# gfxdisp/FovVideoVDP

Measured on AMD Instinct MI355X. Metric: Mpixels/s (test+ref) at 4Kx60f; JOD delta vs reference, higher is better.
Workload: dtype f32

## Files before the change

fovvideovdp_amd/csrc/band2_kernel.hpp:

```cpp
#pragma once
constexpr int F2_PITCH = 54;
constexpr int F2_HL = 6;

struct Band2Args {
    L0Addr A;
    float* Gc;
    int w, h, wb, hb, wc, hc;
    int n_strips, n_chunks, kr;
    int n_big, kr2, n_frames;
    float mulA, mulB;
    const float4* csfA;
    const float4* csfB;
    float y_first, y_inv_step, ly_lo, ly_hi;
    float lg_gain, lg_k, p, q0, q1, beta, lbkg_min, cmax, lg_dmax;
    float* partialA;
    float* partialB;
    int* tickets;
    int n_items;
};

__device__ __forceinline__ v2f dpp_reduce5_pair(v2f acc, v2f v, float u0, float u1, float u3, float u4) {
    float x = acc.x, y = acc.y, l1x, l1y, r1x, r1y, ox, oy;
    asm volatile("s_nop 1\n\t"
                 "v_mov_b32_dpp %2, %8" DPP_SHR "\n\t"
                 "v_mov_b32_dpp %3, %9" DPP_SHR "\n\t"
                 "v_mov_b32_dpp %4, %8" DPP_SHL "\n\t"
                 "v_mov_b32_dpp %5, %9" DPP_SHL "\n\t"
                 "v_fmac_f32_dpp %0, %8, %12" DPP_SHL "\n\t"
                 "v_fmac_f32_dpp %1, %9, %12" DPP_SHL "\n\t"
                 "v_fmac_f32_dpp %0, %2, %10" DPP_SHR "\n\t"
                 "v_fmac_f32_dpp %1, %3, %10" DPP_SHR "\n\t"
                 "v_fmac_f32_dpp %0, %8, %11" DPP_SHR "\n\t"
                 "v_fmac_f32_dpp %1, %9, %11" DPP_SHR "\n\t"
                 "v_fmac_f32_dpp %0, %4, %13" DPP_SHL "\n\t"
                 "v_fmac_f32_dpp %1, %5, %13" DPP_SHL "\n\t"
                 "s_nop 1\n\t"
                 "v_mov_b32_dpp %6, %0 quad_perm:[0,0,2,2] row_mask:0xf bank_mask:0xf bound_ctrl:1\n\t"
                 "v_mov_b32_dpp %7, %1 quad_perm:[0,0,2,2] row_mask:0xf bank_mask:0xf bound_ctrl:1"
                 : "+v"(x), "+v"(y), "=&v"(l1x), "=&v"(l1y), "=&v"(r1x), "=&v"(r1y), "=&v"(ox), "=&v"(oy)
                 : "v"(v.x), "v"(v.y), "v"(u0), "v"(u1), "v"(u3), "v"(u4));
    return v2f{ox, oy};
}
__device__ __forceinline__ v2f dpp_expand2_taps(v2f t, v2f e, float fl, float fr) {
    float x = t.x, y = t.y, l1x, l1y, r1x, r1y;
    asm volatile("s_nop 1\n\t"
                 "v_mov_b32_dpp %2, %6" DPP_SHR "\n\t"
                 "v_mov_b32_dpp %3, %7" DPP_SHR "\n\t"
                 "v_mov_b32_dpp %4, %6" DPP_SHL "\n\t"
                 "v_mov_b32_dpp %5, %7" DPP_SHL "\n\t"
                 "v_fmac_f32_dpp %0, %2, %8" DPP_SHR "\n\t"
                 "v_fmac_f32_dpp %1, %3, %8" DPP_SHR "\n\t"
                 "v_fmac_f32_dpp %0, %4, %9" DPP_SHL "\n\t"
                 "v_fmac_f32_dpp %1, %5, %9" DPP_SHL
                 : "+v"(x), "+v"(y), "=&v"(l1x), "=&v"(l1y), "=&v"(r1x), "=&v"(r1y)
                 : "v"(e.x), "v"(e.y), "v"(fl), "v"(fr));
    return v2f{x, y};
}

constexpr int BAND2_LB = 3;

template <int P, bool INRANGE>
__device__ __forceinline__ void band2_item(const Band2Args& a, const int strip, const int chunk, const int frame, const int lane,
                                           const float4 (*s_csf)[FVVDP_LUT_N], const bool in_step = false) {
    constexpr int HP = P / 2;
    const int blk = chunk * a.n_strips + strip;

    const int w = a.w, h = a.h, wb = a.wb, hb = a.hb, wc = a.wc, hc = a.hc;
    const int J = strip * F2_PITCH - F2_HL + lane;
    const int K = J >> 1;
    const bool jeven = (lane & 1) == 0;
    const bool big = chunk < a.n_big;
    const int ka = big ? chunk * a.kr : a.n_big * a.kr + (chunk - a.n_big) * a.kr2;
    const int kb = min(ka + (big ? a.kr : a.kr2), hc);
    const int ca = 2 * ka, cb = min(2 * kb, hb);
    const bool owned = lane >= F2_HL && lane < F2_HL + F2_PITCH && J < wb;
    const int X0 = 2 * J, X1 = 2 * J + 1;
    const int xc0 = min(max(X0, 0), w - 1), xc1 = min(max(X1, 0), w - 1);
    const bool col1_ok = X1 < w;

    const float K0 = 0.05f, K1 = 0.25f, K2 = 0.4f, K3 = 0.25f, K4 = 0.05f;
    float wq0 = K0, wq1 = K1, wq2 = K2, wq3 = K3, wq4 = K4;
    if (J == 0) { wq2 += K1; wq3 += K0; wq0 = 0.0f; wq1 = 0.0f; }
    if (J == wb - 1) {
        const bool hodd = (h & 1) != 0;
        if (w & 1) { wq3 = 0.0f; wq4 = 0.0f; if (hodd) { wq2 += K3; wq1 += K4; } else { wq2 += K4; } }
        else { wq4 = 0.0f; if (hodd) { wq3 += K3; wq2 += K4; } else { wq3 += K4; } }
    }
    float uq0 = K0, uq1 = K1, uq2 = K2, uq3 = K3, uq4 = K4;
    if (K == 0) { uq2 += K1; uq3 += K0; uq0 = 0.0f; uq1 = 0.0f; }
    if (K == wc - 1) {
        const bool hodd = (hb & 1) != 0;
        if (wb & 1) { uq3 = 0.0f; uq4 = 0.0f; if (hodd) { uq2 += K3; uq1 += K4; } else { uq2 += K4; } }
        else { uq4 = 0.0f; if (hodd) { uq3 += K3; uq2 += K4; } else { uq3 += K4; } }
    }
    const bool at_l = (J <= 0), at_r = (J >= wb - 1);
    const float el = at_l ? 0.0f : 0.1f, er = at_r ? 0.0f : 0.1f;
    const float ec = 0.8f + (at_l ? 0.1f : 0.0f) + (at_r ? 0.1f : 0.0f);
    const float orr = at_r ? 0.0f : 0.5f, oc = at_r ? 1.0f : 0.5f;
    const bool k_l = (K <= 0), k_r = (K >= wc - 1);
    const float fl = (jeven && !k_l) ? 0.1f : 0.0f;
    const float fr = k_r ? 0.0f : (jeven ? 0.1f : 0.5f);
    const float fc = jeven ? (0.8f + (k_l ? 0.1f : 0.0f) + (k_r ? 0.1f : 0.0f)) : (k_r ? 1.0f : 0.5f);

    const float* Ga = l0_frame(a.A, frame);
    float* Gc = a.Gc + (size_t)frame * hc * wc * P;
    const __amdgpu_buffer_rsrc_t Gc_rsrc = level_rsrc(Gc, (unsigned int)(hc * wc * P) * 4u);

    const __amdgpu_buffer_rsrc_t Ga_rsrc = level_rsrc(const_cast<float*>(Ga), (unsigned int)(h * w * P) * 4u);
    const unsigned int col0_b = (unsigned int)xc0 * (P * 4u), col1_b = (unsigned int)xc1 * (P * 4u);
    const unsigned int row_b = (unsigned int)w * (P * 4u);
    auto load_row = [&](int r, Px<P>& p0, Px<P>& p1) {
        int rr = r < 0 ? -1 - r : (r >= h ? 2 * h - 1 - r : r);
        rr = min(max(rr, 0), h - 1);
        const unsigned int so = (unsigned int)rr * row_b;
        p0 = ld_px_buf<P>(Ga_rsrc, col0_b, so);
        p1 = ld_px_buf<P>(Ga_rsrc, col1_b, so);
    };


    Px<P> S[8][2];
    auto coarse_step = [&](auto base) -> Px<P> {
        constexpr int B = decltype(base)::value;
        Px<P>(&W0)[2] = S[(B + 0) & 7]; Px<P>(&W1)[2] = S[(B + 1) & 7]; Px<P>(&W2)[2] = S[(B + 2) & 7];
        Px<P>(&W3)[2] = S[(B + 3) & 7]; Px<P>(&W4)[2] = S[(B + 4) & 7];
        Px<P> c, va, vb;
#pragma unroll
        for (int k = 0; k < HP; ++k) {
            v2f a0 = W0[0].h[k] * K0;
            a0 = pfma(W1[0].h[k], K1, a0);
            a0 = pfma(W2[0].h[k], K2, a0);
            a0 = pfma(W3[0].h[k], K3, a0);
            va.h[k] = pfma(W4[0].h[k], K4, a0);
            v2f b0 = W0[1].h[k] * K0;
            b0 = pfma(W1[1].h[k], K1, b0);
            b0 = pfma(W2[1].h[k], K2, b0);
            b0 = pfma(W3[1].h[k], K3, b0);
            vb.h[k] = pfma(W4[1].h[k], K4, b0);
        }
#pragma unroll
        for (int k = 0; k < HP; ++k) {
            v2f acc = va.h[k] * wq2;
            acc = pfma(vb.h[k], wq3, acc);
            c.h[k] = dpp_reduce_taps(acc, va.h[k], vb.h[k], wq0, wq1, wq4);
        }
        return c;
    };
    float accA[2] = {0.0f, 0.0f}, accB[2] = {0.0f, 0.0f};
    const float lg_base = a.lg_gain;
    const float lg_mask = a.lg_gain + a.lg_k;
    const float lg_bm[2] = {__log2f(a.mulA), __log2f(a.mulB)};
    const float pb = a.p * a.beta, pb_base = lg_base * pb, b_dmax = a.beta * a.lg_dmax, y_off = -a.y_first * a.y_inv_step;

    auto tail = [&](const Px<P>& g, const Px<P>& e, bool valid, const int band, float (&acc)[2]) {
        const float lb = INRANGE ? e.h[0].y : fmaxf(e.h[0].y, a.lbkg_min);
        const float dcap = a.cmax * lb;
        v2f d[HP];
#pragma unroll
        for (int k = 0; k < HP; ++k) {
            if constexpr (INRANGE) d[k] = v2f{g.h[k].x - e.h[k].x, g.h[k].y - e.h[k].y};
            else d[k] = v2f{fminf(g.h[k].x - e.h[k].x, dcap), fminf(g.h[k].y - e.h[k].y, dcap)};
        }
        const float llb = fast_log2(lb);
        const float yq = INRANGE ? llb : __builtin_amdgcn_fmed3f(llb, a.ly_lo, a.ly_hi);
        const float t = fmaf(yq, a.y_inv_step, y_off);
        float4 r;
        float f;
        if constexpr (INRANGE) {
            r = s_csf[band][floor_to_int(t)];
            f = __builtin_amdgcn_fractf(t);
        } else {
            const float fi = __builtin_amdgcn_fmed3f(floorf(t), 0.0f, (float)(FVVDP_LUT_N - 2));
            r = s_csf[band][(int)fi];
            f = t - fi;
        }
        const float slog0 = fmaf(f, r.z, r.x), slog1 = fmaf(f, r.w, r.y);
        const float vm = valid ? 1.0f : 0.0f;
        const float lcn = lg_bm[band] - llb;
        if constexpr (HP == 2) {
            const v2f sl = v2f{slog0, slog1};
            const v2f A = pfma(sl, pb, splat(fmaf(lcn, pb, pb_base)));
            const v2f lsm = sl + splat(lcn + lg_mask);
            const v2f ldiff = v2f{fast_log2(fabsf(d[0].x - d[0].y)), fast_log2(fabsf(d[1].x - d[1].y))};
            const v2f lmin = v2f{fast_log2(fminf(fabsf(d[0].x), fabsf(d[0].y))), fast_log2(fminf(fabsf(d[1].x), fabsf(d[1].y)))};
            const v2f ldb = pfma(ldiff, pb, A);
            const v2f lm = (lmin + lsm) * v2f{a.q0, a.q1};
            const v2f one_mq = v2f{fast_exp2(lm.x), fast_exp2(lm.y)} + splat(1.0f);
            const v2f tb = pfma(v2f{fast_log2(one_mq.x), fast_log2(one_mq.y)}, -a.beta, ldb);
            const v2f bl = v2f{fminf(tb.x, b_dmax), fminf(tb.y, b_dmax)};
            const v2f term = v2f{fast_exp2(bl.x), fast_exp2(bl.y)};
            const v2f av = __builtin_elementwise_fma(term, splat(vm), v2f{acc[0], acc[1]});
            acc[0] = av.x;
            acc[1] = av.y;
        } else {
            const float dT = d[0].x, dR = d[0].y;
            const float ls = slog0 + lcn;
            const float ld = a.p * (fast_log2(fabsf(dT - dR)) + (ls + lg_base));
            const float mq = fast_exp2(a.q0 * (fast_log2(fminf(fabsf(dT), fabsf(dR))) + (ls + lg_mask)));
            const float ldd = fminf(ld - fast_log2(1.0f + mq), a.lg_dmax);
            acc[0] = fmaf(fast_exp2(a.beta * ldd), vm, acc[0]);
        }
// ... 60 lines not shown
            e0.h[k] = dpp_expand2_taps(evE.h[k] * fc, evE.h[k], fl, fr);
            e1.h[k] = dpp_expand2_taps(evO.h[k] * fc, evO.h[k], fl, fr);
        }
        tail(g0, e0, owned && row0 < hb, 1, accB);
        tail(g1, e1, owned && (row0 + 1) < hb, 1, accB);
    };

    auto stage = [&](auto basea, auto baseb, int k) {
        constexpr int BA = decltype(basea)::value, BB = decltype(baseb)::value;
        Px<P> Be, Bo;
        if (in_step) __builtin_amdgcn_s_barrier();
        {
            const int c = 2 * k;
            load_row(2 * c + 5, S[(BA + 5) & 7][0], S[(BA + 5) & 7][1]);
            load_row(2 * c + 6, S[(BA + 6) & 7][0], S[(BA + 6) & 7][1]);
            Be = coarse_step(basea);
            if (c + 1 >= hb) Be = R[4];
            if (c >= ca && c < cb) band_a_rows(basea, c, R[3], R[4], Be);
        }
        {
            const int c = 2 * k + 1;
            load_row(2 * c + 5, S[(BB + 5) & 7][0], S[(BB + 5) & 7][1]);
            load_row(2 * c + 6, S[(BB + 6) & 7][0], S[(BB + 6) & 7][1]);
            Bo = coarse_step(baseb);
            if (c + 1 >= hb) Bo = (c + 1 == hb) ? Be : R[3];
            if (c >= ca && c < cb) band_a_rows(baseb, c, R[4], Be, Bo);
        }
        R[0] = R[2];
        R[1] = R[3];
        R[2] = R[4];
        R[3] = Be;
        R[4] = Bo;
        if (k == 0) {
            R[0] = R[3];
            R[1] = R[2];
        }
        Px<P> Cn;
#pragma unroll
        for (int q = 0; q < HP; ++q) {
            v2f v = R[0].h[q] * K0;
            v = pfma(R[1].h[q], K1, v);
            v = pfma(R[2].h[q], K2, v);
            v = pfma(R[3].h[q], K3, v);
            v = pfma(R[4].h[q], K4, v);
            Cn.h[q] = dpp_reduce5_pair(v * uq2, v, uq0, uq1, uq3, uq4);
        }
        st_px(Gc_rsrc, (k >= ka && k < kb && owned && jeven && K < wc) ? (unsigned int)(k * wc + K) * (P * 4u) : FVVDP_NO_STORE, Cn);
        CH[0] = CH[1];
        CH[1] = CH[2];
        CH[2] = Cn;
        if (k == 0) CH[1] = Cn;
        const int row0 = 2 * k - 2;
        if (row0 >= ca && row0 < cb) band_b_rows(R[0], R[1], row0);
    };
    {
        int k = ks;
        for (; k + 1 <= kend; k += 2) {
            stage(I0(), I2(), k);
            stage(I4(), I6(), k + 1);
        }
        if (k <= kend) stage(I0(), I2(), k);
    }
    if (last_chunk) {
        const int row0 = 2 * hc - 2;
        CH[0] = CH[1];
        CH[1] = CH[2];
        if (row0 >= ca && row0 < cb) band_b_rows(R[2], R[3], row0);
    }

    const float a0 = wave_sum(accA[0]), a1 = wave_sum(accA[1]);
    const float b0 = wave_sum(accB[0]), b1 = wave_sum(accB[1]);
    if (lane == 0) {
        const size_t o = ((size_t)frame * (a.n_strips * a.n_chunks) + blk) * 2;
        a.partialA[o] = a0;
        a.partialA[o + 1] = a1;
        a.partialB[o] = b0;
        a.partialB[o + 1] = b1;
    }
}

#define BAND2_WPB_MAX 4

template <int P, bool INRANGE = false>
__global__ __launch_bounds__(64 * BAND2_WPB_MAX, BAND2_LB) void band2_kernel(const Band2Args a) {
    __shared__ float4 s_csf[2][FVVDP_LUT_N];
    __shared__ int s_item[2];
    const int lane = threadIdx.x & 63;
    const int wpb = (int)(blockDim.x >> 6);
    const int n_groups = a.n_strips / wpb;
    const int first = n_groups * a.n_big * a.n_frames;
    int bid;
    bool tall;
    if (a.tickets) {
        if (threadIdx.x == 0) {
#if defined(__gfx942__) || defined(__gfx950__)
            const int x = (int)__builtin_amdgcn_s_getreg((4 - 1) << 11 | 20) & 7;
#else
            const int x = (int)(blockIdx.x & 7);
#endif
            const int nbp[2] = {first, a.n_items - first};
            int item = -1, ph_found = 0;
            for (int k = 0; k < 16 && item < 0; ++k) {
                const int ph = (k == 0) ? 0 : (k == 1 ? 1 : (k < 9 ? 0 : 1));
                const int y = (k < 2) ? x : ((x + (k < 9 ? k - 1 : k - 8)) & 7);
                const int q8 = nbp[ph] >> 3, r8 = nbp[ph] & 7, cnt = q8 + (y < r8 ? 1 : 0);
                int* tk = a.tickets + ph * 8 + y;
                if (__hip_atomic_load(tk, __ATOMIC_RELAXED, __HIP_MEMORY_SCOPE_AGENT) >= cnt) continue;
                const int t = atomicAdd(tk, 1);
                if (t < cnt) { item = y * q8 + min(y, r8) + t; ph_found = ph; }
            }
            s_item[0] = item;
            s_item[1] = ph_found;
        }
        __syncthreads();
        bid = s_item[0];
        tall = s_item[1] == 0;
        if (bid < 0) return;
    } else {
        int v = (int)blockIdx.x, nb = first;
        tall = v < first;
        if (!tall) { v -= first; nb = (int)gridDim.x - first; }
        const int q8 = nb >> 3, r8 = nb & 7, x = v & 7;
        bid = x * q8 + min(x, r8) + (v >> 3);
    }
    const int group = bid % n_groups;
    bid /= n_groups;
    const int per_frame = tall ? a.n_big : a.n_chunks - a.n_big;
    const int chunk = (tall ? 0 : a.n_big) + bid % per_frame;
    const int frame = bid / per_frame;
    const int strip = group * wpb + (int)(threadIdx.x >> 6);
    if (threadIdx.x < FVVDP_LUT_N) {
        s_csf[0][threadIdx.x] = a.csfA[threadIdx.x];
        s_csf[1][threadIdx.x] = a.csfB[threadIdx.x];
    }
    __syncthreads();
    band2_item<P, INRANGE>(a, strip, chunk, frame, lane, s_csf, wpb > 1);
}
```

fovvideovdp_amd/csrc/fvvdp_hip.hip:

```cpp
#include <hip/hip_runtime.h>
#include <hip/hip_fp16.h>

#include <algorithm>
#include <cmath>
#include <cfloat>
#include <cstdarg>
#include <cstdio>
#include <cstdlib>
#include <cstring>
#include <type_traits>
#include <vector>

#include "fvvdp_hip.h"
#include "fvvdp_hip_images.h"
#include "fvvdp_hip_gaze.h"
#include "fvvdp_hip_tests.h"
#include "fvvdp_hip_ref_grad.h"
#include "fvvdp_hip_params.h"
#include "fvvdp_hip_diffmap.h"

static thread_local char g_err[512] = "";

static int fail(int code, const char* fmt, ...) {
    va_list ap;
    va_start(ap, fmt);
    vsnprintf(g_err, sizeof(g_err), fmt, ap);
    va_end(ap);
    return code;
}

#define HIP_TRY(expr)                                                                              \
    do {                                                                                           \
        hipError_t e_ = (expr);                                                                    \
        if (e_ != hipSuccess) return fail(FVVDP_EHIP, "%s failed: %s", #expr, hipGetErrorString(e_)); \
    } while (0)

extern "C" const char* fvvdp_last_error(void) { return g_err; }
int fvvdp_fail_from(int code, const char* msg) { return fail(code, "%s", msg); }

#include "device_common.hpp"
#include "temporal_kernels.hpp"
#include "temporal_launch.hpp"
#include "band_kernel.hpp"
#include "band2_kernel.hpp"
#include "aux_kernels.hpp"
#include "multigaze_kernel.hpp"
#include "multitest_kernel.hpp"
#include "still_kernels.hpp"
#include "psnr_kernel.hpp"
#include "resize_kernels.hpp"

struct CtxEnv {
    bool alloc_malloc = false;
    size_t vmm_chunk = 0;
    int probe_n = -1;
    int probe_extra = -1;
    float probe_mixed = 6.75f;
    bool inrange_off = false;
    int fuse_mode = -1;
    int band2_kr = 0, band2_kr2 = -1, band2_wpb = 0;
    int k1_ticket = -1;
    int level0_split = -1;
    int band2_ticket = -1;
    bool temporal_scalar = false;
    bool debug_variant = false;
    int gaze_group = 0;
    int band_cr = 0;
    int tests_group = 0;
    bool yuv_general = false;
};
static CtxEnv read_env() {
    CtxEnv e;
    auto num = [](const char* name, int dflt) { const char* v = getenv(name); return (v && v[0]) ? atoi(v) : dflt; };
    if (const char* v = getenv("FVVDP_ALLOC")) e.alloc_malloc = strcmp(v, "malloc") == 0;
    e.vmm_chunk = (size_t)(num("FVVDP_VMM_CHUNK_MB", 0) > 0 ? num("FVVDP_VMM_CHUNK_MB", 0) : 0) << 20;
    e.probe_n = num("FVVDP_PLACEMENT_PROBE", -1);
    e.probe_extra = num("FVVDP_PLACEMENT_EXTRA", -1);
    if (const char* v = getenv("FVVDP_PLACEMENT_MIXED_TBS")) e.probe_mixed = (float)atof(v);
    if (const char* v = getenv("FVVDP_BAND_INRANGE")) e.inrange_off = v[0] == '0';
    if (const char* v = getenv("FVVDP_BAND_FUSE")) e.fuse_mode = (v[0] == '0' || v[0] == '1') ? v[0] - '0' : -1;
    e.band2_kr = num("FVVDP_BAND2_KR", 0);
    e.band2_kr2 = num("FVVDP_BAND2_KR2", -1);
    e.band2_wpb = num("FVVDP_BAND2_WPB", 0);
    if (const char* v = getenv("FVVDP_K1_TICKET")) e.k1_ticket = v[0] != '0' ? 1 : 0;
    if (const char* v = getenv("FVVDP_BAND2_TICKET")) e.band2_ticket = v[0] != '0' ? 1 : 0;
    if (const char* v = getenv("FVVDP_LEVEL0_SPLIT")) e.level0_split = v[0] != '0' ? 1 : 0;
    e.temporal_scalar = getenv("FVVDP_TEMPORAL_SCALAR") != nullptr;
    e.debug_variant = getenv("FVVDP_DEBUG_VARIANT") != nullptr;
    e.yuv_general = getenv("FVVDP_YUV_GENERAL_MATRIX") != nullptr;
    e.gaze_group = num("FVVDP_GAZE_GROUP", 0);
    e.band_cr = num("FVVDP_BAND_CR", 0);
    e.tests_group = num("FVVDP_TESTS_GROUP", 0);
    return e;
}

struct VmmBlock {
    void* ptr;
    size_t size;
    std::vector<hipMemGenericAllocationHandle_t> handles;
};
struct fvvdp_ctx {
    CtxEnv env;
    int W = 0, H = 0, n_bands = 0, P = 0, max_frames = 0;
    fvvdp_params prm{};
    double rho_band[FVVDP_MAX_BANDS + 1]{};
    int lw[FVVDP_MAX_BANDS + 1]{}, lh[FVVDP_MAX_BANDS + 1]{};
    float* level[FVVDP_MAX_BANDS + 1]{};
    float* level0_hi = nullptr;
    int sel_phase = 9;
    int sel_n = 0;
    int sel_kept = -1;
    float sel_us[8] = {0, 0, 0, 0, 0, 0, 0, 0};
    int level0_kind = 0;
    int level0_kind_hi = -1;
    long long n_sync = 0, n_alloc = 0, n_free = 0;
    bool created = false;
    bool lum_known = false;
    int lum_state = 0;
    int lum_hold = 0;
    int lum_top = 0;
    float lum_lo = 0.0f, lum_hi = 0.0f, lum_width = 0.0f;
    float* partial = nullptr;
    long long partial_off[FVVDP_MAX_BANDS]{};
    int max_blk[FVVDP_MAX_BANDS]{};
    int* d_ticket = nullptr;
    size_t partial_floats = 0;
    float4* csf = nullptr;
    float4* csf_y = nullptr;
    bool csf_set = false;
    float y_first = 0, y_inv_step = 0, y_lo = 0, y_hi = 0;
    std::vector<float> h_lut3[2];
    float h_axes[3][FVVDP_LUT_N]{};
    float* d_axes = nullptr;
    float4* sublut[FVVDP_MAX_BANDS]{};
    float4* rmap[FVVDP_MAX_BANDS]{};
    int sub_rw[FVVDP_MAX_BANDS]{}, sub_ilo[FVVDP_MAX_BANDS]{};
    fvvdp_geom sub_geom{};
    const float* map_vx[FVVDP_MAX_BANDS]{};
    const float* map_vy[FVVDP_MAX_BANDS]{};
    const float* map_rm[FVVDP_MAX_BANDS]{};
    float map_rm_max[FVVDP_MAX_BANDS]{}, map_rm_min[FVVDP_MAX_BANDS]{};
    bool maps_set = false;
    float* slope[FVVDP_MAX_BANDS]{};
    bool sub_valid = false;
    float rho_lo = 0, rho_hi = 0, ecc_lo = 0, ecc_hi = 0;
    bool lut3_set[2] = {false, false};
    float* d_fix = nullptr;
    float* d_taps = nullptr;
    int* d_idx = nullptr;
    float* lum_buf = nullptr;
    size_t lum_floats = 0;
    float* heat[FVVDP_MAX_BANDS + 1]{};
    unsigned int* colour_ws = nullptr;
    size_t scratch = 0;
    std::vector<VmmBlock> vmm;
    long long wave_capacity = 4096;
    long long wave_capacity2 = 4096;
    bool timing = false;
    std::vector<std::pair<hipEvent_t, hipEvent_t>> ev[FVVDP_MAX_BANDS + 2];
    float t_ms[FVVDP_MAX_BANDS + 2]{};
    int t_cnt[FVVDP_MAX_BANDS + 2]{};
};

static const size_t VMM_MIN_BYTES = (size_t)16 << 20;
static const size_t VMM_BIG_BYTES = (size_t)256 << 20;

static int vmm_alloc(fvvdp_ctx* c, void** out, size_t bytes);
static void vmm_free_all(fvvdp_ctx* c);

template <typename T>
static int dev_alloc(fvvdp_ctx* c, T** p, size_t count) {
    void* q = nullptr;
    const size_t bytes = count * sizeof(T);
    if (!c->env.alloc_malloc && bytes >= VMM_MIN_BYTES && vmm_alloc(c, &q, bytes) == FVVDP_OK) {
    } else {
        q = nullptr;
        (void)hipGetLastError();
        hipError_t e = hipMalloc(&q, bytes);
        if (e != hipSuccess) return fail(FVVDP_ENOMEM, "hipMalloc(%zu bytes) failed: %s", bytes, hipGetErrorString(e));
    }
    *p = reinterpret_cast<T*>(q);
    c->scratch += bytes;
    if (c->created) c->n_alloc += 1;
    return FVVDP_OK;
}

static L0Addr level_addr(const fvvdp_ctx* c, int L, int slot0) {
    L0Addr a;
    const size_t fr = (size_t)c->lw[L] * c->lh[L] * c->P;
    a.lo = c->level[L];
    a.slot0 = slot0;
    if (L == 0 && c->level0_hi) { a.hi = c->level0_hi; a.half_stride = fr; }
    else { a.hi = c->level[L] + fr; a.half_stride = 2 * fr; }
    return a;
}

struct Timed {
    fvvdp_ctx* c;
    int id;
    hipStream_t st;
    hipEvent_t e0 = nullptr, e1 = nullptr;
    Timed(fvvdp_ctx* c_, int id_, hipStream_t st_) : c(c_), id(id_), st(st_) {
        if (c->timing) {
            (void)hipEventCreate(&e0);
            (void)hipEventCreate(&e1);
            (void)hipEventRecord(e0, st);
        }
    }
    ~Timed() {
        if (c->timing) {
// ... 35 lines not shown
        if (e == hipSuccess) mapped = (i + 1) * chunk;
    }
    hipMemAccessDesc acc;
    memset(&acc, 0, sizeof(acc));
    acc.location = prop.location;
    acc.flags = hipMemAccessFlagsProtReadWrite;
    if (e == hipSuccess) e = hipMemSetAccess(b.ptr, size, &acc, 1);
    if (e != hipSuccess) {
        if (mapped) (void)hipMemUnmap(b.ptr, mapped);
        for (auto h : b.handles) (void)hipMemRelease(h);
        (void)hipMemAddressFree(b.ptr, size);
        return fail(FVVDP_ENOMEM, "mapping %zu chunks of %zu bytes failed: %s", n, chunk, hipGetErrorString(e));
    }
    c->vmm.push_back(b);
    *out = b.ptr;
    return FVVDP_OK;
}

static bool vmm_owns(const fvvdp_ctx* c, const void* p) {
    for (const VmmBlock& b : c->vmm)
        if (b.ptr == p) return true;
    return false;
}

static void dev_free(fvvdp_ctx* c, void* p) {
    if (p && !vmm_owns(c, p)) (void)hipFree(p);
}

static void vmm_free_one(fvvdp_ctx* c, void* p) {
    for (size_t i = 0; i < c->vmm.size(); ++i)
        if (c->vmm[i].ptr == p) {
            VmmBlock& b = c->vmm[i];
            (void)hipMemUnmap(b.ptr, b.size);
            for (auto h : b.handles) (void)hipMemRelease(h);
            (void)hipMemAddressFree(b.ptr, b.size);
            c->vmm.erase(c->vmm.begin() + (long)i);
            return;
        }
}

static void vmm_free_all(fvvdp_ctx* c) {
    for (VmmBlock& b : c->vmm) {
        (void)hipMemUnmap(b.ptr, b.size);
        for (auto h : b.handles) (void)hipMemRelease(h);
        (void)hipMemAddressFree(b.ptr, b.size);
    }
    c->vmm.clear();
}

static int band_strips(int wc) { return wc <= 62 ? 1 : 1 + (wc - 62 + STRIP_J - 1) / STRIP_J; }

static int band2_strips(int wb) { return (wb + F2_PITCH - 1) / F2_PITCH; }

static void chunking2(int hc, int n_strips, int n, long long capacity, int kr_override, int& n_chunks, int& kr) {
    double best = 1e300;
    kr = hc;
    for (int cand = 1; cand <= hc; ++cand) {
        const long long chunks = (hc + cand - 1) / cand;
        const long long waves = (long long)n * n_strips * chunks;
        const long long rounds = (waves + capacity - 1) / capacity;
        const double cost = (double)rounds * (2.0 * cand + 9.0) * (1.0 + 1e-4 * (double)chunks);
        if (cost < best) { best = cost; kr = cand; }
    }
    if (kr_override >= 1) kr = kr_override > hc ? hc : kr_override;
    n_chunks = (hc + kr - 1) / kr;
}

static void chunking(int hc, int n_strips, int n, long long capacity, int& n_chunks, int& cr) {
    double best = 1e300;
    cr = hc;
    for (int cand = 2; cand <= hc || cand == 2; ++cand) {
        const int c = cand > hc ? hc : cand;
        const long long chunks = (hc + c - 1) / c;
        const long long waves = (long long)n * n_strips * chunks;
        const long long rounds = (waves + capacity - 1) / capacity;
        const double cost = (double)rounds * ((double)c + 8.0) * (1.0 + 1e-4 * (double)chunks);
        if (cost < best) { best = cost; cr = c; }
        if (cand >= hc) break;
    }
    n_chunks = (hc + cr - 1) / cr;
}

static void choose_level0(fvvdp_ctx* c);

static bool band2_takes(const fvvdp_ctx* c, int b) {
    const bool big = (long long)c->lw[b] * c->lh[b] >= 500000;
    return (big || c->env.fuse_mode == 1) && b + 1 < c->n_bands && c->lw[b + 1] >= 4 && c->lh[b + 1] >= 4 &&
           c->lw[b + 2] >= 2 && c->lh[b + 2] >= 2;
}

static void band2_plan(const fvvdp_ctx* c, int b, int plan_n, int& n_strips, int& n_chunks, int& kr, int& n_big, int& kr2_out) {
    const int hc = c->lh[b + 2];
    n_strips = band2_strips(c->lw[b + 1]);
    chunking2(hc, n_strips, plan_n, c->wave_capacity2, c->env.band2_kr, n_chunks, kr);
    n_big = n_chunks;
    kr2_out = kr;
    const long long waves = (long long)plan_n * n_strips * n_chunks;
    int kr2 = (waves >= 2 * c->wave_capacity2 && n_chunks >= 3 && kr >= 16) ? (kr + 3) / 4 : 0;
    if (c->env.band2_kr2 >= 0) kr2 = c->env.band2_kr2;
    if (kr2 >= 1 && kr2 < kr && n_chunks >= 2) {
        n_big = n_chunks - 1;
        kr2_out = kr2;
        n_chunks = n_big + (hc - n_big * kr + kr2 - 1) / kr2;
    }
}

extern "C" int fvvdp_ctx_create(fvvdp_ctx** out, int width, int height, int n_bands, int planes, int max_frames,
                                const double* h_rho_band, const fvvdp_params* prm) {
    if (!out || !prm || !h_rho_band) return fail(FVVDP_EINVAL, "null argument");
    if (planes != 2 && planes != 4) return fail(FVVDP_EINVAL, "planes must be 2 (image) or 4 (video), got %d", planes);
    if (n_bands < 1 || n_bands > FVVDP_MAX_BANDS) return fail(FVVDP_EINVAL, "n_bands %d out of range", n_bands);
    if (max_frames < 1) return fail(FVVDP_EINVAL, "max_frames must be >= 1");
    if (width < 4 || height < 4) return fail(FVVDP_EINVAL, "frame %dx%d too small", width, height);
    fvvdp_ctx* c = new fvvdp_ctx();
    c->env = read_env();
    c->W = width;
    c->H = height;
    c->n_bands = n_bands;
    c->P = planes;
    c->max_frames = max_frames;
    c->prm = *prm;
    int w = width, h = height;
    for (int i = 0; i <= n_bands; ++i) {
        c->lw[i] = w;
        c->lh[i] = h;
        c->rho_band[i] = h_rho_band[i];
        if (i < n_bands && (w < 2 || h < 2)) {
            delete c;
            return fail(FVVDP_EINVAL, "pyramid level %d is %dx%d: too many bands for this frame size", i, w, h);
        }
        w = (w + 1) / 2;
        h = (h + 1) / 2;
    }
    int rc = FVVDP_OK;
    for (int i = 0; i <= n_bands && rc == FVVDP_OK; ++i) {
        rc = dev_alloc(c, &c->level[i], (size_t)max_frames * c->lw[i] * c->lh[i] * planes);
    }
    size_t off = 0;
    for (int b = 0; b < n_bands; ++b) {
        const int n_strips = band_strips(c->lw[b + 1]);
        const int max_chunks = (c->lh[b + 1] + 1) / 2;
        c->max_blk[b] = n_strips * max_chunks;
    }
    for (int b = 0; b + 1 < n_bands; ++b) {
        const int blk2 = band2_strips(c->lw[b + 1]) * c->lh[b + 2];
        if (blk2 > c->max_blk[b]) c->max_blk[b] = blk2;
        if (blk2 > c->max_blk[b + 1]) c->max_blk[b + 1] = blk2;
    }
    for (int b = 0; b < n_bands; ++b) {
        c->partial_off[b] = (long long)off;
        off += (size_t)max_frames * c->max_blk[b] * 2;
    }
    c->partial_floats = off;
    if (rc == FVVDP_OK) rc = dev_alloc(c, &c->partial, off);
    if (rc == FVVDP_OK) {
        float* q = nullptr;
        rc = dev_alloc(c, &q, 16);
        c->d_ticket = reinterpret_cast<int*>(q);
    }
    if (rc == FVVDP_OK) rc = dev_alloc(c, &c->csf, (size_t)n_bands * FVVDP_LUT_N);
    if (rc == FVVDP_OK) rc = dev_alloc(c, &c->csf_y, (size_t)FVVDP_LUT_N);
    if (rc == FVVDP_OK) rc = dev_alloc(c, &c->d_fix, (size_t)max_frames * 2);
    if (rc == FVVDP_OK) rc = dev_alloc(c, &c->d_taps, (size_t)2 * FVVDP_MAX_TAPS);
    if (rc == FVVDP_OK) rc = dev_alloc(c, &c->d_idx, (size_t)max_frames + FVVDP_MAX_TAPS);
    if (rc != FVVDP_OK) {
        fvvdp_ctx_destroy(c);
        return rc;
    }
    {
        int dev = 0, cus = 256, per_cu = 16;
        if (hipGetDevice(&dev) == hipSuccess) {
            hipDeviceProp_t prop;
            if (hipGetDeviceProperties(&prop, dev) == hipSuccess) cus = prop.multiProcessorCount;
        }
        hipError_t e = (planes == 4)
            ? hipOccupancyMaxActiveBlocksPerMultiprocessor(&per_cu, band_kernel<4, false, 0>, 64, 0)
            : hipOccupancyMaxActiveBlocksPerMultiprocessor(&per_cu, band_kernel<2, false, 0>, 64, 0);
        if (e != hipSuccess || per_cu < 1) per_cu = 16;
        c->wave_capacity = (long long)per_cu * cus;
        int per_cu2 = 16;
        e = (planes == 4) ? hipOccupancyMaxActiveBlocksPerMultiprocessor(&per_cu2, band2_kernel<4, false>, 64, 0)
                          : hipOccupancyMaxActiveBlocksPerMultiprocessor(&per_cu2, band2_kernel<2, false>, 64, 0);
        if (e != hipSuccess || per_cu2 < 1) per_cu2 = 16;
        c->wave_capacity2 = (long long)per_cu2 * cus;
    }
    choose_level0(c);
    if (!c->level[0]) {
        fvvdp_ctx_destroy(c);
        return fail(FVVDP_ENOMEM, "no device memory for pyramid level 0");
    }
    c->created = true;
    *out = c;
    return FVVDP_OK;
}

extern "C" void fvvdp_ctx_destroy(fvvdp_ctx* c) {
    if (!c) return;
    (void)hipDeviceSynchronize();
    for (int i = 0; i <= FVVDP_MAX_BANDS; ++i)
        dev_free(c, c->level[i]);
    dev_free(c, c->level0_hi);
    dev_free(c, c->partial);
    dev_free(c, c->d_ticket);
    if (c->csf) (void)hipFree(c->csf);
    if (c->csf_y) (void)hipFree(c->csf_y);
    for (int i = 0; i <= FVVDP_MAX_BANDS; ++i)
        dev_free(c, c->heat[i]);
    if (c->colour_ws) (void)hipFree(c->colour_ws);
    if (c->d_fix) (void)hipFree(c->d_fix);
    if (c->d_taps) (void)hipFree(c->d_taps);
// ... 800 lines not shown
    hipStream_t st = reinterpret_cast<hipStream_t>(stream);
    if (fov) {
        HIP_TRY(hipMemcpyAsync(c->d_fix, h_fixation, sizeof(float) * 2 * n, hipMemcpyHostToDevice, st));
        int rc = build_sublut(c, geom, st);
        if (rc != FVVDP_OK) return rc;
    }
    FinalizeArgs fa;
    memset(&fa, 0, sizeof(fa));
    bool any_maps = false;
    if (maps)
        for (int b = 0; b < c->n_bands; ++b) any_maps = any_maps || maps[b].d_D || maps[b].d_contrast || maps[b].d_lbkg || maps[b].d_S;
    const int fuse_mode = c->env.fuse_mode;
    const bool fuse_ok = !fov && !any_maps && fuse_mode != 0;
    for (int b = 0; b < c->n_bands; ++b) {
        if (fuse_ok && band2_takes(c, b)) {
            Band2Args a;
            memset(&a, 0, sizeof(a));
            a.A = level_addr(c, b, b == 0 ? slot0 : 0);
            a.Gc = c->level[b + 2];
            a.w = c->lw[b];
            a.h = c->lh[b];
            a.wb = c->lw[b + 1];
            a.hb = c->lh[b + 1];
            a.wc = c->lw[b + 2];
            a.hc = c->lh[b + 2];
            band2_plan(c, b, plan_n, a.n_strips, a.n_chunks, a.kr, a.n_big, a.kr2);
            a.n_frames = n;
            a.mulA = (b == 0) ? 1.0f : 2.0f;
            a.mulB = 2.0f;
            a.csfA = c->csf + (size_t)b * FVVDP_LUT_N;
            a.csfB = c->csf + (size_t)(b + 1) * FVVDP_LUT_N;
            a.y_first = c->y_first;
            a.y_inv_step = c->y_inv_step;
            a.ly_lo = log2f(c->y_lo);
            a.ly_hi = log2f(c->y_hi);
            a.lg_gain = log2f(c->prm.sens_gain);
            a.lg_k = log2f(c->prm.mask_k);
            a.p = c->prm.mask_p;
            a.q0 = c->prm.mask_q[0];
            a.q1 = c->prm.mask_q[1];
            a.beta = c->prm.beta;
            a.lbkg_min = c->prm.lbkg_min;
            a.cmax = c->prm.contrast_max;
            a.lg_dmax = log2f(c->prm.d_max);
            a.partialA = c->partial + c->partial_off[b];
            a.partialB = c->partial + c->partial_off[b + 1];
            const int nblk = a.n_strips * a.n_chunks;
            if (nblk > c->max_blk[b] || nblk > c->max_blk[b + 1]) return fail(FVVDP_ESTATE, "internal: partial buffer too small");
            {
                Timed tm(c, 1 + b, st);
                const bool inrange = clamps_never_bind(c, b, 2);
                int wpb = (a.w >= 2560 && a.n_strips % BAND2_WPB_MAX == 0) ? BAND2_WPB_MAX : 1;
                { const int v = c->env.band2_wpb; if (v >= 1 && v <= BAND2_WPB_MAX && a.n_strips % v == 0) wpb = v; }
                const int n_items = (a.n_strips / wpb) * a.n_chunks * n;
                const long long waves2 = (long long)n * a.n_strips * a.n_chunks;
                bool tickets = c->d_ticket && (c->env.band2_ticket == 1 ||
                                               (c->env.band2_ticket != 0 && waves2 >= 2 * c->wave_capacity2 && wpb == BAND2_WPB_MAX && a.w >= 2560));
                if (tickets && hipMemsetAsync(c->d_ticket, 0, 16 * sizeof(int), st) != hipSuccess) { (void)hipGetLastError(); tickets = false; }
                a.n_items = n_items;
                a.tickets = tickets ? c->d_ticket : nullptr;
                const int n_wg = tickets ? ((n_items + n_items / 8 + 7) / 8 * 8) : n_items;
                const dim3 grid2((unsigned int)n_wg), block2(64 * wpb);
                if (c->env.debug_variant)
                    fprintf(stderr, "fvvdp: levels %d+%d: band2_kernel<%d, %s>, luminance range %s [%g, %g], widest plane range %g, %d waves per workgroup"
                                    ", n_strips %d, kr %d, kr2 %d, n_big %d, n_chunks %d, tickets %s\n",
                                 b, b + 1, c->P, inrange ? "true" : "false", c->lum_state == 1 ? "known" : "unknown", c->lum_lo, c->lum_hi, c->lum_width, wpb,
                                 a.n_strips, a.kr, a.kr2, a.n_big, a.n_chunks, tickets ? "on" : "off");
                if (c->P == 4) {
                    if (inrange) hipLaunchKernelGGL((band2_kernel<4, true>), grid2, block2, 0, st, a);
                    else hipLaunchKernelGGL((band2_kernel<4, false>), grid2, block2, 0, st, a);
                } else {
                    if (inrange) hipLaunchKernelGGL((band2_kernel<2, true>), grid2, block2, 0, st, a);
                    else hipLaunchKernelGGL((band2_kernel<2, false>), grid2, block2, 0, st, a);
                }
            }
            for (int bb = b; bb <= b + 1; ++bb) {
                fa.nblk[bb] = nblk;
                fa.off[bb] = c->partial_off[bb];
                fa.npx[bb] = (float)c->lw[bb] * (float)c->lh[bb];
            }
            ++b;
            continue;
        }
        BandArgs a;
        fill_band_args(c, b, slot0, plan_n, fov, geom, a);
        a.partial = c->partial + c->partial_off[b];
        bool dbg = false;
        if (maps) {
            a.dD = maps[b].d_D;
            a.dC = maps[b].d_contrast;
            a.dL = maps[b].d_lbkg;
            a.dS = maps[b].d_S;
            dbg = a.dD || a.dC || a.dL || a.dS;
        }
        const int nblk = a.n_strips * a.n_chunks;
        if (nblk > c->max_blk[b]) return fail(FVVDP_ESTATE, "internal: partial buffer too small");
        a.n_items = nblk * n;
        if (c->env.debug_variant) debug_band_line(c, b, a, n, dbg, fov);
        {
            Timed tm(c, 1 + b, st);
            if (c->P == 4) launch_band<4>(a, nblk * n, dbg, fov, st, c->slope[b]);
            else launch_band<2>(a, nblk * n, dbg, fov, st, c->slope[b]);
        }
        fa.nblk[b] = nblk;
        fa.off[b] = c->partial_off[b];
        fa.npx[b] = (float)a.w * (float)a.h;
    }
    fa.partial = c->partial;
    fa.Q = d_Q;
    fa.n_bands = c->n_bands;
    fa.n = n;
    fa.q_stride = q_stride;
    fa.q_col0 = q_col0;
    fa.tc = c->P / 2;
    fa.inv_beta = 1.0f / c->prm.beta;
    {
        Timed tm(c, 1 + c->n_bands, st);
        const int total = c->n_bands * 2 * n;
        hipLaunchKernelGGL(finalize_kernel, dim3(total), dim3(64), 0, st, fa);
    }
// ... 782 lines not shown
```

Baseline: 259,600.

## Merge adjacent band2 row chunks into multi-chunk runs chosen by a makespan planner

Lets a single band2 work item process a run of consecutive row chunks. It flushes per-chunk partial sums at the chunk seams, so the overlap and startup rows are not recomputed for each chunk. A host-side planner simulates the makespan of candidate run layouts against wave capacity and picks the best one, memoised per geometry. The ticket scheduler and the plain scheduler are generalised to up to four phases. The trade is fewer, longer items and so possibly worse load balance, plus extra host planning work on first use.

```diff
diff --git a/fovvideovdp_amd/csrc/band2_kernel.hpp b/fovvideovdp_amd/csrc/band2_kernel.hpp
--- a/fovvideovdp_amd/csrc/band2_kernel.hpp
+++ b/fovvideovdp_amd/csrc/band2_kernel.hpp
@@ -17,6 +17,8 @@
     float* partialB;
     int* tickets;
     int n_items;
+    int n_phases;
+    int run_first[BAND2_MAX_PHASES], run_len[BAND2_MAX_PHASES], run_count[BAND2_MAX_PHASES], ph_items[BAND2_MAX_PHASES];
 };
 
 __device__ __forceinline__ v2f dpp_reduce5_pair(v2f acc, v2f v, float u0, float u1, float u3, float u4) {
@@ -60,18 +62,18 @@
 constexpr int BAND2_LB = 3;
 
 template <int P, bool INRANGE>
-__device__ __forceinline__ void band2_item(const Band2Args& a, const int strip, const int chunk, const int frame, const int lane,
+__device__ __forceinline__ void band2_item(const Band2Args& a, const int strip, const int chunk, const int run_len, const int frame, const int lane,
                                            const float4 (*s_csf)[FVVDP_LUT_N], const bool in_step = false) {
     constexpr int HP = P / 2;
-    const int blk = chunk * a.n_strips + strip;
 
     const int w = a.w, h = a.h, wb = a.wb, hb = a.hb, wc = a.wc, hc = a.hc;
     const int J = strip * F2_PITCH - F2_HL + lane;
     const int K = J >> 1;
     const bool jeven = (lane & 1) == 0;
-    const bool big = chunk < a.n_big;
-    const int ka = big ? chunk * a.kr : a.n_big * a.kr + (chunk - a.n_big) * a.kr2;
-    const int kb = min(ka + (big ? a.kr : a.kr2), hc);
+    auto chunk_row0 = [&](int c) { return min(c <= a.n_big ? c * a.kr : a.n_big * a.kr + (c - a.n_big) * a.kr2, hc); };
+    const int chunk_last = chunk + run_len - 1;
+    const int ka = chunk_row0(chunk);
+    const int kb = chunk_row0(chunk_last + 1);
     const int ca = 2 * ka, cb = min(2 * kb, hb);
     const bool owned = lane >= F2_HL && lane < F2_HL + F2_PITCH && J < wb;
     const int X0 = 2 * J, X1 = 2 * J + 1;
@@ -146,6 +148,17 @@
         return c;
     };
     float accA[2] = {0.0f, 0.0f}, accB[2] = {0.0f, 0.0f};
+    auto flush = [&](float (&acc)[2], float* partial, int c) {
+        const float s0 = wave_sum(acc[0]), s1 = wave_sum(acc[1]);
+        if (lane == 0) {
+            const size_t o = ((size_t)frame * (a.n_strips * a.n_chunks) + (c * a.n_strips + strip)) * 2;
+            partial[o] = s0;
+            partial[o + 1] = s1;
+        }
+        acc[0] = 0.0f;
+        acc[1] = 0.0f;
+    };
+    int cur = chunk, seam = chunk_row0(chunk + 1);
     const float lg_base = a.lg_gain;
     const float lg_mask = a.lg_gain + a.lg_k;
     const float lg_bm[2] = {__log2f(a.mulA), __log2f(a.mulB)};
@@ -312,6 +325,14 @@
         if (k == 0) CH[1] = Cn;
         const int row0 = 2 * k - 2;
         if (row0 >= ca && row0 < cb) band_b_rows(R[0], R[1], row0);
+        if (cur < chunk_last) {
+            if (k == seam) {
+                flush(accB, a.partialB, cur);
+                ++cur;
+                seam = chunk_row0(cur + 1);
+            }
+            if (k + 1 == seam && cur < chunk_last) flush(accA, a.partialA, cur);
+        }
     };
     {
         int k = ks;
@@ -328,15 +349,8 @@
         if (row0 >= ca && row0 < cb) band_b_rows(R[2], R[3], row0);
     }
 
-    const float a0 = wave_sum(accA[0]), a1 = wave_sum(accA[1]);
-    const float b0 = wave_sum(accB[0]), b1 = wave_sum(accB[1]);
-    if (lane == 0) {
-        const size_t o = ((size_t)frame * (a.n_strips * a.n_chunks) + blk) * 2;
-        a.partialA[o] = a0;
-        a.partialA[o + 1] = a1;
-        a.partialB[o] = b0;
-        a.partialB[o + 1] = b1;
-    }
+    flush(accA, a.partialA, chunk_last);
+    flush(accB, a.partialB, chunk_last);
 }
 
 #define BAND2_WPB_MAX 4
@@ -348,9 +362,7 @@
     const int lane = threadIdx.x & 63;
     const int wpb = (int)(blockDim.x >> 6);
     const int n_groups = a.n_strips / wpb;
-    const int first = n_groups * a.n_big * a.n_frames;
-    int bid;
-    bool tall;
+    int bid, ph;
     if (a.tickets) {
         if (threadIdx.x == 0) {
 #if defined(__gfx942__) || defined(__gfx950__)
@@ -358,35 +370,37 @@
 #else
             const int x = (int)(blockIdx.x & 7);
 #endif
-            const int nbp[2] = {first, a.n_items - first};
+            const int np = a.n_phases;
             int item = -1, ph_found = 0;
-            for (int k = 0; k < 16 && item < 0; ++k) {
-                const int ph = (k == 0) ? 0 : (k == 1 ? 1 : (k < 9 ? 0 : 1));
-                const int y = (k < 2) ? x : ((x + (k < 9 ? k - 1 : k - 8)) & 7);
-                const int q8 = nbp[ph] >> 3, r8 = nbp[ph] & 7, cnt = q8 + (y < r8 ? 1 : 0);
-                int* tk = a.tickets + ph * 8 + y;
+            for (int k = 0; k < 8 * np && item < 0; ++k) {
+                const int p = k < np ? k : (k - np) / 7;
+                const int y = k < np ? x : ((x + 1 + (k - np) % 7) & 7);
+                const int nb = a.ph_items[p];
+                const int q8 = nb >> 3, r8 = nb & 7, cnt = q8 + (y < r8 ? 1 : 0);
+                int* tk = a.tickets + p * 8 + y;
                 if (__hip_atomic_load(tk, __ATOMIC_RELAXED, __HIP_MEMORY_SCOPE_AGENT) >= cnt) continue;
                 const int t = atomicAdd(tk, 1);
-                if (t < cnt) { item = y * q8 + min(y, r8) + t; ph_found = ph; }
+                if (t < cnt) { item = y * q8 + min(y, r8) + t; ph_found = p; }
             }
             s_item[0] = item;
             s_item[1] = ph_found;
         }
         __syncthreads();
         bid = s_item[0];
-        tall = s_item[1] == 0;
+        ph = s_item[1];
         if (bid < 0) return;
     } else {
-        int v = (int)blockIdx.x, nb = first;
-        tall = v < first;
-        if (!tall) { v -= first; nb = (int)gridDim.x - first; }
+        int v = (int)blockIdx.x;
+        ph = 0;
+        while (ph + 1 < a.n_phases && v >= a.ph_items[ph]) v -= a.ph_items[ph++];
+        const int nb = a.ph_items[ph];
         const int q8 = nb >> 3, r8 = nb & 7, x = v & 7;
         bid = x * q8 + min(x, r8) + (v >> 3);
     }
     const int group = bid % n_groups;
     bid /= n_groups;
-    const int per_frame = tall ? a.n_big : a.n_chunks - a.n_big;
-    const int chunk = (tall ? 0 : a.n_big) + bid % per_frame;
+    const int per_frame = a.run_count[ph], run_len = a.run_len[ph];
+    const int chunk = a.run_first[ph] + (bid % per_frame) * run_len;
     const int frame = bid / per_frame;
     const int strip = group * wpb + (int)(threadIdx.x >> 6);
     if (threadIdx.x < FVVDP_LUT_N) {
@@ -394,5 +408,5 @@
         s_csf[1][threadIdx.x] = a.csfB[threadIdx.x];
     }
     __syncthreads();
-    band2_item<P, INRANGE>(a, strip, chunk, frame, lane, s_csf, wpb > 1);
+    band2_item<P, INRANGE>(a, strip, chunk, run_len, frame, lane, s_csf, wpb > 1);
 }
diff --git a/fovvideovdp_amd/csrc/band2_runs.hpp b/fovvideovdp_amd/csrc/band2_runs.hpp
--- /dev/null
+++ b/fovvideovdp_amd/csrc/band2_runs.hpp
@@ -0,0 +1,191 @@
+#pragma once
+#include <functional>
+#include <map>
+
+struct Band2Grid {
+    int hc, kr, kr2, n_big, n_chunks;
+};
+
+inline int band2_chunk_row0(const Band2Grid& g, int c) {
+    const int r = c <= g.n_big ? c * g.kr : g.n_big * g.kr + (c - g.n_big) * g.kr2;
+    return r < g.hc ? r : g.hc;
+}
+
+constexpr int BAND2_ITEM_STARTUP = 9;
+
+inline void chunking2(int hc, int n_strips, int n, long long capacity, int kr_override, int& n_chunks, int& kr) {
+    double best = 1e300;
+    kr = hc;
+    for (int cand = 1; cand <= hc; ++cand) {
+        const long long chunks = (hc + cand - 1) / cand;
+        const long long waves = (long long)n * n_strips * chunks;
+        const long long rounds = (waves + capacity - 1) / capacity;
+        const double cost = (double)rounds * (2.0 * cand + (double)BAND2_ITEM_STARTUP) * (1.0 + 1e-4 * (double)chunks);
+        if (cost < best) { best = cost; kr = cand; }
+    }
+    if (kr_override >= 1) kr = kr_override > hc ? hc : kr_override;
+    n_chunks = (hc + kr - 1) / kr;
+}
+
+inline Band2Grid band2_grid(int hc, int n_strips, int n, long long wave_capacity, int kr_override, int kr2_override) {
+    Band2Grid g;
+    g.hc = hc;
+    chunking2(hc, n_strips, n, wave_capacity, kr_override, g.n_chunks, g.kr);
+    g.n_big = g.n_chunks;
+    g.kr2 = g.kr;
+    const long long waves = (long long)n * n_strips * g.n_chunks;
+    int kr2 = (waves >= 2 * wave_capacity && g.n_chunks >= 3 && g.kr >= 16) ? (g.kr + 3) / 4 : 0;
+    if (kr2_override >= 0) kr2 = kr2_override;
+    if (kr2 >= 1 && kr2 < g.kr && g.n_chunks >= 2) {
+        g.n_big = g.n_chunks - 1;
+        g.kr2 = kr2;
+        g.n_chunks = g.n_big + (hc - g.n_big * g.kr + kr2 - 1) / kr2;
+    }
+    return g;
+}
+
+constexpr int BAND2_MAX_PHASES = 4;
+
+struct Band2Runs {
+    int n_phases;
+    int first[BAND2_MAX_PHASES], len[BAND2_MAX_PHASES], count[BAND2_MAX_PHASES];
+};
+
+inline int band2_run_rows(const Band2Grid& g, int first, int len) { return band2_chunk_row0(g, first + len) - band2_chunk_row0(g, first); }
+
+inline int band2_runs_per_column(const Band2Runs& r) {
+    int n = 0;
+    for (int p = 0; p < r.n_phases; ++p) n += r.count[p];
+    return n;
+}
+
+inline bool band2_runs_equal(const Band2Runs& a, const Band2Runs& b) {
+    if (a.n_phases != b.n_phases) return false;
+    for (int p = 0; p < a.n_phases; ++p)
+        if (a.first[p] != b.first[p] || a.len[p] != b.len[p] || a.count[p] != b.count[p]) return false;
+    return true;
+}
+
+inline void band2_runs_sort(const Band2Grid& g, Band2Runs& r) {
+    for (int i = 1; i < r.n_phases; ++i)
+        for (int j = i; j > 0 && band2_run_rows(g, r.first[j], r.len[j]) > band2_run_rows(g, r.first[j - 1], r.len[j - 1]); --j) {
+            int t;
+            t = r.first[j]; r.first[j] = r.first[j - 1]; r.first[j - 1] = t;
+            t = r.len[j]; r.len[j] = r.len[j - 1]; r.len[j - 1] = t;
+            t = r.count[j]; r.count[j] = r.count[j - 1]; r.count[j - 1] = t;
+        }
+}
+
+inline Band2Runs band2_runs_single(const Band2Grid& g) {
+    Band2Runs r{};
+    r.n_phases = 1;
+    r.first[0] = 0; r.len[0] = 1; r.count[0] = g.n_big;
+    if (g.n_big < g.n_chunks) {
+        r.n_phases = 2;
+        r.first[1] = g.n_big; r.len[1] = 1; r.count[1] = g.n_chunks - g.n_big;
+    }
+    return r;
+}
+
+inline Band2Runs band2_runs_fixed(const Band2Grid& g, int m) {
+    if (m <= 1) return band2_runs_single(g);
+    if (m > g.n_chunks) m = g.n_chunks;
+    Band2Runs r{};
+    r.n_phases = 1;
+    r.first[0] = 0; r.len[0] = m; r.count[0] = g.n_chunks / m;
+    const int rem = g.n_chunks % m;
+    if (rem) {
+        r.n_phases = 2;
+        r.first[1] = g.n_chunks - rem; r.len[1] = rem; r.count[1] = 1;
+    }
+    band2_runs_sort(g, r);
+    return r;
+}
+
+inline long long band2_runs_makespan(const Band2Grid& g, const Band2Runs& r, long long columns, long long capacity) {
+    std::map<long long, long long> slots;
+    slots[0] = capacity < 1 ? 1 : capacity;
+    long long end = 0;
+    for (int p = 0; p < r.n_phases; ++p) {
+        std::map<long long, long long, std::greater<long long>> cls;
+        for (int j = 0; j < r.count[p]; ++j)
+            cls[2LL * band2_run_rows(g, r.first[p] + j * r.len[p], r.len[p]) + BAND2_ITEM_STARTUP] += columns;
+        for (const auto& kv : cls) {
+            const long long cost = kv.first;
+            long long n = kv.second;
+            while (n > 0) {
+                auto it = slots.begin();
+                const long long t = it->first, k = it->second < n ? it->second : n;
+                if (k == it->second) slots.erase(it);
+                else it->second -= k;
+                slots[t + cost] += k;
+                if (t + cost > end) end = t + cost;
+                n -= k;
+            }
+        }
+    }
+    return end;
+}
+
+constexpr int BAND2_RUN_MIN_ROUNDS = 4;
+
+namespace band2_detail {
+struct Search {
+    const Band2Grid& g;
+    long long columns, capacity;
+    Band2Runs best;
+    long long best_t, single_t;
+    Band2Runs cur;
+    void consider() {
+        Band2Runs r = cur;
+        band2_runs_sort(g, r);
+        if ((2LL * band2_run_rows(g, r.first[0], r.len[0]) + BAND2_ITEM_STARTUP) * BAND2_RUN_MIN_ROUNDS > single_t) return;
+        const long long t = band2_runs_makespan(g, r, columns, capacity);
+        if (t < best_t) { best_t = t; best = r; }
+    }
+    void rec(int at) {
+        if (at == g.n_chunks) { consider(); return; }
+        if (cur.n_phases == BAND2_MAX_PHASES) return;
+        const int left = g.n_chunks - at, p = cur.n_phases;
+        for (int len = 1; len <= left; ++len) {
+            if (p > 0 && len == cur.len[p - 1]) continue;
+            for (int count = 1; count * len <= left; ++count) {
+                if (p == BAND2_MAX_PHASES - 1 && count * len != left) continue;
+                cur.first[p] = at; cur.len[p] = len; cur.count[p] = count;
+                cur.n_phases = p + 1;
+                rec(at + count * len);
+                cur.n_phases = p;
+            }
+        }
+    }
+};
+}
+
+inline Band2Runs band2_runs_plan(const Band2Grid& g, int n_groups, int n_frames, long long capacity, int fixed = 0) {
+    if (fixed >= 1) return band2_runs_fixed(g, fixed);
+    const Band2Runs single = band2_runs_single(g);
+    const long long columns = (long long)n_groups * n_frames;
+    if (columns * g.n_chunks <= capacity) return single;
+    const long long single_t = band2_runs_makespan(g, single, columns, capacity);
+    band2_detail::Search s{g, columns, capacity, single, single_t, single_t, Band2Runs{}};
+    if (g.n_chunks <= 12) {
+        s.rec(0);
+    } else {
+        for (int m = 2; m <= 8; ++m) {
+            s.cur = band2_runs_fixed(g, m);
+            s.consider();
+            if (g.n_big < g.n_chunks && m <= g.n_big) {
+                Band2Runs& c = s.cur;
+                c = Band2Runs{};
+                c.first[0] = 0; c.len[0] = m; c.count[0] = g.n_big / m;
+                c.n_phases = 1;
+                const int rem = g.n_big % m;
+                if (rem) { c.first[1] = g.n_big - rem; c.len[1] = rem; c.count[1] = 1; c.n_phases = 2; }
+                c.first[c.n_phases] = g.n_big; c.len[c.n_phases] = 1; c.count[c.n_phases] = g.n_chunks - g.n_big;
+                ++c.n_phases;
+                s.consider();
+            }
+        }
+    }
+    return s.best;
+}
diff --git a/fovvideovdp_amd/csrc/fvvdp_hip.hip b/fovvideovdp_amd/csrc/fvvdp_hip.hip
--- a/fovvideovdp_amd/csrc/fvvdp_hip.hip
+++ b/fovvideovdp_amd/csrc/fvvdp_hip.hip
@@ -42,6 +42,7 @@
 #include "temporal_kernels.hpp"
 #include "temporal_launch.hpp"
 #include "band_kernel.hpp"
+#include "band2_runs.hpp"
 #include "band2_kernel.hpp"
 #include "aux_kernels.hpp"
 #include "multigaze_kernel.hpp"
@@ -62,6 +63,7 @@
     int k1_ticket = -1;
     int level0_split = -1;
     int band2_ticket = -1;
+    int band2_runs = 0;
     bool temporal_scalar = false;
     bool debug_variant = false;
     int gaze_group = 0;
@@ -82,6 +84,7 @@
     e.band2_kr = num("FVVDP_BAND2_KR", 0);
     e.band2_kr2 = num("FVVDP_BAND2_KR2", -1);
     e.band2_wpb = num("FVVDP_BAND2_WPB", 0);
+    e.band2_runs = num("FVVDP_BAND2_RUNS", 0);
     if (const char* v = getenv("FVVDP_K1_TICKET")) e.k1_ticket = v[0] != '0' ? 1 : 0;
     if (const char* v = getenv("FVVDP_BAND2_TICKET")) e.band2_ticket = v[0] != '0' ? 1 : 0;
     if (const char* v = getenv("FVVDP_LEVEL0_SPLIT")) e.level0_split = v[0] != '0' ? 1 : 0;
@@ -156,6 +159,8 @@
     std::vector<VmmBlock> vmm;
     long long wave_capacity = 4096;
     long long wave_capacity2 = 4096;
+    struct { Band2Grid grid; int n_groups, n_frames; Band2Runs runs; bool valid = false; } runs_memo[4];
+    int runs_memo_next = 0;
     bool timing = false;
     std::vector<std::pair<hipEvent_t, hipEvent_t>> ev[FVVDP_MAX_BANDS + 2];
     float t_ms[FVVDP_MAX_BANDS + 2]{};
@@ -297,20 +302,6 @@
 
 static int band2_strips(int wb) { return (wb + F2_PITCH - 1) / F2_PITCH; }
 
-static void chunking2(int hc, int n_strips, int n, long long capacity, int kr_override, int& n_chunks, int& kr) {
-    double best = 1e300;
-    kr = hc;
-    for (int cand = 1; cand <= hc; ++cand) {
-        const long long chunks = (hc + cand - 1) / cand;
-        const long long waves = (long long)n * n_strips * chunks;
-        const long long rounds = (waves + capacity - 1) / capacity;
-        const double cost = (double)rounds * (2.0 * cand + 9.0) * (1.0 + 1e-4 * (double)chunks);
-        if (cost < best) { best = cost; kr = cand; }
-    }
-    if (kr_override >= 1) kr = kr_override > hc ? hc : kr_override;
-    n_chunks = (hc + kr - 1) / kr;
-}
-
 static void chunking(int hc, int n_strips, int n, long long capacity, int& n_chunks, int& cr) {
     double best = 1e300;
     cr = hc;
@@ -335,19 +326,27 @@
 }
 
 static void band2_plan(const fvvdp_ctx* c, int b, int plan_n, int& n_strips, int& n_chunks, int& kr, int& n_big, int& kr2_out) {
-    const int hc = c->lh[b + 2];
     n_strips = band2_strips(c->lw[b + 1]);
-    chunking2(hc, n_strips, plan_n, c->wave_capacity2, c->env.band2_kr, n_chunks, kr);
-    n_big = n_chunks;
-    kr2_out = kr;
-    const long long waves = (long long)plan_n * n_strips * n_chunks;
-    int kr2 = (waves >= 2 * c->wave_capacity2 && n_chunks >= 3 && kr >= 16) ? (kr + 3) / 4 : 0;
-    if (c->env.band2_kr2 >= 0) kr2 = c->env.band2_kr2;
-    if (kr2 >= 1 && kr2 < kr && n_chunks >= 2) {
-        n_big = n_chunks - 1;
-        kr2_out = kr2;
-        n_chunks = n_big + (hc - n_big * kr + kr2 - 1) / kr2;
-    }
+    const Band2Grid g = band2_grid(c->lh[b + 2], n_strips, plan_n, c->wave_capacity2, c->env.band2_kr, c->env.band2_kr2);
+    n_chunks = g.n_chunks;
+    kr = g.kr;
+    n_big = g.n_big;
+    kr2_out = g.kr2;
+}
+
+static Band2Runs band2_runs_of(fvvdp_ctx* c, const Band2Args& a, int n_groups, int n_frames, int wpb) {
+    const Band2Grid g{a.hc, a.kr, a.kr2, a.n_big, a.n_chunks};
+    for (auto& m : c->runs_memo)
+        if (m.valid && m.n_groups == n_groups && m.n_frames == n_frames && m.grid.hc == g.hc && m.grid.kr == g.kr && m.grid.kr2 == g.kr2 &&
+            m.grid.n_big == g.n_big && m.grid.n_chunks == g.n_chunks)
+            return m.runs;
+    auto& m = c->runs_memo[c->runs_memo_next++ & 3];
+    m.grid = g;
+    m.n_groups = n_groups;
+    m.n_frames = n_frames;
+    m.runs = band2_runs_plan(g, n_groups, n_frames, c->wave_capacity2 / wpb, c->env.band2_runs);
+    m.valid = true;
+    return m.runs;
 }
 
 extern "C" int fvvdp_ctx_create(fvvdp_ctx** out, int width, int height, int n_bands, int planes, int max_frames,
@@ -400,7 +399,7 @@
     if (rc == FVVDP_OK) rc = dev_alloc(c, &c->partial, off);
     if (rc == FVVDP_OK) {
         float* q = nullptr;
-        rc = dev_alloc(c, &q, 16);
+        rc = dev_alloc(c, &q, 8 * BAND2_MAX_PHASES);
         c->d_ticket = reinterpret_cast<int*>(q);
     }
     if (rc == FVVDP_OK) rc = dev_alloc(c, &c->csf, (size_t)n_bands * FVVDP_LUT_N);
@@ -1307,11 +1306,21 @@
                 const bool inrange = clamps_never_bind(c, b, 2);
                 int wpb = (a.w >= 2560 && a.n_strips % BAND2_WPB_MAX == 0) ? BAND2_WPB_MAX : 1;
                 { const int v = c->env.band2_wpb; if (v >= 1 && v <= BAND2_WPB_MAX && a.n_strips % v == 0) wpb = v; }
-                const int n_items = (a.n_strips / wpb) * a.n_chunks * n;
+                const int n_groups = a.n_strips / wpb;
+                const Band2Runs runs = band2_runs_of(c, a, n_groups, n, wpb);
+                int n_items = 0;
+                a.n_phases = runs.n_phases;
+                for (int p = 0; p < runs.n_phases; ++p) {
+                    a.run_first[p] = runs.first[p];
+                    a.run_len[p] = runs.len[p];
+                    a.run_count[p] = runs.count[p];
+                    a.ph_items[p] = n_groups * runs.count[p] * n;
+                    n_items += a.ph_items[p];
+                }
                 const long long waves2 = (long long)n * a.n_strips * a.n_chunks;
                 bool tickets = c->d_ticket && (c->env.band2_ticket == 1 ||
                                                (c->env.band2_ticket != 0 && waves2 >= 2 * c->wave_capacity2 && wpb == BAND2_WPB_MAX && a.w >= 2560));
-                if (tickets && hipMemsetAsync(c->d_ticket, 0, 16 * sizeof(int), st) != hipSuccess) { (void)hipGetLastError(); tickets = false; }
+                if (tickets && hipMemsetAsync(c->d_ticket, 0, 8 * BAND2_MAX_PHASES * sizeof(int), st) != hipSuccess) { (void)hipGetLastError(); tickets = false; }
                 a.n_items = n_items;
                 a.tickets = tickets ? c->d_ticket : nullptr;
                 const int n_wg = tickets ? ((n_items + n_items / 8 + 7) / 8 * 8) : n_items;
@@ -1321,6 +1330,11 @@
                                     ", n_strips %d, kr %d, kr2 %d, n_big %d, n_chunks %d, tickets %s\n",
                                  b, b + 1, c->P, inrange ? "true" : "false", c->lum_state == 1 ? "known" : "unknown", c->lum_lo, c->lum_hi, c->lum_width, wpb,
                                  a.n_strips, a.kr, a.kr2, a.n_big, a.n_chunks, tickets ? "on" : "off");
+                if (c->env.debug_variant) {
+                    fprintf(stderr, "fvvdp: levels %d+%d: band2 runs: %d items, %d per column, phases", b, b + 1, n_items, band2_runs_per_column(runs));
+                    for (int p = 0; p < runs.n_phases; ++p) fprintf(stderr, " [first %d len %d count %d]", runs.first[p], runs.len[p], runs.count[p]);
+                    fprintf(stderr, "\n");
+                }
                 if (c->P == 4) {
                     if (inrange) hipLaunchKernelGGL((band2_kernel<4, true>), grid2, block2, 0, st, a);
                     else hipLaunchKernelGGL((band2_kernel<4, false>), grid2, block2, 0, st, a);
```

After: 254,400. 2.0% lower.
